# nightgoodl/ovmono3d

Measured on AMD Instinct MI355X. Metric: images/sec/GPU @512x512 DINOv2-L SFP; AP3D delta vs reference, higher is better.
Workload: dtype f16x3; 1 GPU; DINOv2 vitl14 + SFP + ROIHeads3DGDINO (native GroundingDINO Swin-B/BERT-base, 900 queries, 6 categories -> NMS) + ROIAlign + CubeHead + decode, batch 1/GPU, 512x512 synthetic -> network res 532 -> canvas 896 (T=4097), random-init weights (seed 0); precision=f16x3, parallelism=dp1 (image-sharded, no data-path collective)

## Files before the change

### ovmono3d_amd/csrc/attn.hip

```cpp
#include "kernels.hpp"
#include "attn_tail.hpp"
#include <type_traits>

namespace ovm {

__device__ __forceinline__ int swz128(int row, int chunk) { return chunk ^ ((row >> 1) & 7); }

__device__ __forceinline__ void split2_pk(float p0, float p1, uint32_t& hp, uint32_t& lp) {
  float d0, d1;
  asm("s_nop 0\n\tv_cvt_pk_f16_f32 %0, %1, %2" : "=v"(hp) : "v"(p0), "v"(p1));
  asm("v_fma_mix_f32 %0, %1, 1.0, -%2 op_sel:[0,0,0] op_sel_hi:[0,0,1]" : "=v"(d0) : "v"(p0), "v"(hp));
  asm("v_fma_mix_f32 %0, %1, 1.0, -%2 op_sel:[0,0,1] op_sel_hi:[0,0,1]" : "=v"(d1) : "v"(p1), "v"(hp));
  asm("v_cvt_pk_f16_f32 %0, %1, %2" : "=v"(lp) : "v"(d0), "v"(d1));
}
__device__ __forceinline__ uint32_t cvt2_pk(float p0, float p1) {
  uint32_t hp;
  asm("s_nop 0\n\tv_cvt_pk_f16_f32 %0, %1, %2" : "=v"(hp) : "v"(p0), "v"(p1));
  return hp;
}
typedef uint32_t u32x4 __attribute__((ext_vector_type(4)));

template <int N> __device__ __forceinline__ void wait_vmcnt_n() {
  __builtin_amdgcn_s_waitcnt((N & 0xF) | (7 << 4) | (15 << 8) | ((N >> 4) << 14));
}

constexpr float kPShift = 14.0f;

#ifndef OVM_ATTN_ILV
#define OVM_ATTN_ILV 0
#endif
#ifndef OVM_ATTN_RD
#define OVM_ATTN_RD 3
#endif
template <int NPASS, int NW>
__global__ __launch_bounds__(64 * NW, NW == 4 ? 2 : 1) void attn_kernel(const AttnParams p) {
  extern __shared__ __attribute__((aligned(16))) char smem[];
  if ((int)blockIdx.x >= p.main_blocks) { attn_tail_any<NPASS>(p, (int)blockIdx.x - p.main_blocks, smem); return; }
  static_assert(NW == 4 || NW == 8, "4 or 8 waves");
  const unsigned long long t_wg0 = p.stamps ? __builtin_amdgcn_s_memtime() : 0ull;
  constexpr int PART = 64 * 128;
  constexpr int SLOT = PART * ((NPASS == 3) ? 2 : 1);
  constexpr int RD = OVM_ATTN_RD;
  char* const Kring = smem;
  char* const Vring = smem + RD * SLOT;
  const int tid = threadIdx.x, lane = tid & 63, wave = tid >> 6;
  const int nqb = (p.Tq + 32 * NW - 1) / (32 * NW);
  const int bid = xcd_remap(blockIdx.x, p.main_blocks);
  const int bh = bid / nqb, qb = bid - bh * nqb;
  const int b = bh / p.heads, head = bh - b * p.heads;
  const int T = p.T;
  const size_t qk_base = (size_t)bh * T * 64;
  const size_t v_base = (size_t)bh * 64 * p.Tpad;
  const int h = lane >> 5, r = lane & 31;

  int q = qb * (32 * NW) + wave * 32 + r;
  const bool q_ok = q < p.Tq;
  if (!q_ok) q = T - 1;
  half8 qh[4], ql[4];
#pragma unroll
  for (int s = 0; s < 4; ++s) {
    qh[s] = *(const half8*)(p.Qhi + qk_base + (size_t)q * 64 + 16 * s + 8 * h);
    if (NPASS == 3) ql[s] = *(const half8*)(p.Qlo + qk_base + (size_t)q * 64 + 16 * s + 8 * h);
  }

  constexpr int PPW = 8 / NW;
  int drow[PPW], dch[PPW];
#pragma unroll
  for (int t = 0; t < PPW; ++t) {
    drow[t] = (wave + NW * t) * 8 + (lane >> 3);
    dch[t] = swz128(drow[t], lane & 7) * 8;
  }
  auto stageK = [&](int slot, int it) {
    char* base = Kring + slot * SLOT;
    const int k0 = it * 64;
#pragma unroll
    for (int t = 0; t < PPW; ++t) {
      int key = k0 + drow[t]; if (key > T - 1) key = T - 1;
      const size_t o = qk_base + (size_t)key * 64 + dch[t];
      glds16(p.Khi + o, base + (wave + NW * t) * 1024);
      if (NPASS == 3) glds16(p.Klo + o, base + PART + (wave + NW * t) * 1024);
    }
  };
  auto stageV = [&](int slot, int it) {
    char* base = Vring + slot * SLOT;
    const int k0 = it * 64;
#pragma unroll
    for (int t = 0; t < PPW; ++t) {
      const size_t o = v_base + (size_t)drow[t] * p.Tpad + k0 + dch[t];
      glds16(p.Vhi + o, base + (wave + NW * t) * 1024);
      if (NPASS == 3) glds16(p.Vlo + o, base + PART + (wave + NW * t) * 1024);
    }
  };
  auto qk = [&](const char* kb, f32x16* s) {
#if OVM_ATTN_ILV
#pragma unroll
    for (int i = 0; i < 2; ++i)
#pragma unroll
      for (int e = 0; e < 16; ++e) s[i][e] = 0.f;
#pragma unroll
    for (int st = 0; st < 4; ++st) {
      half8 kh[2], kl[2];
#pragma unroll
      for (int i = 0; i < 2; ++i) {
        const int row = 32 * i + r;
        const int off = row * 128 + swz128(row, 2 * st + h) * 16;
        kh[i] = *(const half8*)(kb + off);
        if (NPASS == 3) kl[i] = *(const half8*)(kb + PART + off);
      }
      if (NPASS == 3) {
#pragma unroll
        for (int i = 0; i < 2; ++i) s[i] = __builtin_amdgcn_mfma_f32_32x32x16_f16(kl[i], qh[st], s[i], 0, 0, 0);
#pragma unroll
        for (int i = 0; i < 2; ++i) s[i] = __builtin_amdgcn_mfma_f32_32x32x16_f16(kh[i], ql[st], s[i], 0, 0, 0);
      }
#pragma unroll
      for (int i = 0; i < 2; ++i) s[i] = __builtin_amdgcn_mfma_f32_32x32x16_f16(kh[i], qh[st], s[i], 0, 0, 0);
    }
#else
#pragma unroll
    for (int i = 0; i < 2; ++i) {
#pragma unroll
      for (int e = 0; e < 16; ++e) s[i][e] = 0.f;
      const int row = 32 * i + r;
#pragma unroll
      for (int st = 0; st < 4; ++st) {
        const int off = row * 128 + swz128(row, 2 * st + h) * 16;
        const half8 kh = *(const half8*)(kb + off);
        if (NPASS == 3) {
          const half8 kl = *(const half8*)(kb + PART + off);
          s[i] = __builtin_amdgcn_mfma_f32_32x32x16_f16(kl, qh[st], s[i], 0, 0, 0);
          s[i] = __builtin_amdgcn_mfma_f32_32x32x16_f16(kh, ql[st], s[i], 0, 0, 0);
        }
        s[i] = __builtin_amdgcn_mfma_f32_32x32x16_f16(kh, qh[st], s[i], 0, 0, 0);
      }
    }
#endif
  };

  f32x16 o0[2];
#pragma unroll
  for (int t = 0; t < 2; ++t)
#pragma unroll
    for (int i = 0; i < 16; ++i) o0[t][i] = 0.f;
  float m_run = -1e30f, l_run = 0.f;

  const int nt = (T + 63) >> 6;
  stageK(0, 0);
  stageV(0, 0);
  if (nt > 1) stageK(1, 1);
  if (RD >= 3) {
    if (nt > 2) stageK(2, 2);
    if (nt > 1) stageV(1, 1);
  }
  if (RD >= 4) {
    if (nt > 3) stageK(3, 3);
    if (nt > 2) stageV(2, 2);
  }
  int prev_mine = 0;
  asm volatile("s_waitcnt vmcnt(0)" ::: "memory");
  __syncthreads();
  f32x16 sc[2], sn[2];
  qk(Kring, sc);
  __syncthreads();

  auto tile = [&](int it, auto last_tag) {
    constexpr bool LAST = decltype(last_tag)::value;
    if (!LAST) {
      if (it + RD < nt) stageK(it % RD, it + RD);
      if (it + RD - 1 < nt) stageV((it + RD - 1) % RD, it + RD - 1);
      qk(Kring + ((it + 1) % RD) * SLOT, sn);
    }
    const int kbase = it * 64;
    if (LAST) {
#pragma unroll
      for (int i = 0; i < 2; ++i)
#pragma unroll
        for (int e = 0; e < 16; ++e) {
          const int key = kbase + 32 * i + (e & 3) + 8 * (e >> 2) + 4 * h;
          if (key >= T) sc[i][e] = -1e30f;
        }
    }
    float mx = -1e30f;
#pragma unroll
    for (int i = 0; i < 2; ++i)
#pragma unroll
      for (int e = 0; e < 16; ++e) mx = fmaxf(mx, sc[i][e]);
    mx = fmaxf(mx, __shfl_xor(mx, 32, 64));
    const float m_new = fmaxf(m_run, mx);
    const float alpha = __builtin_amdgcn_exp2f(m_run - m_new);
    m_run = m_new;
    typedef float f32x2 __attribute__((ext_vector_type(2)));
    const f32x2 shift2 = {kPShift - m_new, kPShift - m_new};
    f32x2 psum2 = {0.f, 0.f};
    u32x4 phu[2][2], plu[2][2];
#pragma unroll
    for (int i = 0; i < 2; ++i)
#pragma unroll
      for (int sp = 0; sp < 2; ++sp) {
#pragma unroll
        for (int e = 0; e < 8; e += 2) {
          f32x2 d = {sc[i][8 * sp + e], sc[i][8 * sp + e + 1]};
          d += shift2;
// ... 22 lines not shown
          const int off = row * 128 + swz128(row, 4 * i + 2 * sp + h) * 16;
          vh[t] = *(const half8*)(vb + off);
          if (NPASS == 3) vl[t] = *(const half8*)(vb + PART + off);
        }
        if (NPASS == 3) {
#pragma unroll
          for (int t = 0; t < 2; ++t) o0[t] = __builtin_amdgcn_mfma_f32_32x32x16_f16(vl[t], __builtin_bit_cast(half8, phu[i][sp]), o0[t], 0, 0, 0);
#pragma unroll
          for (int t = 0; t < 2; ++t) o0[t] = __builtin_amdgcn_mfma_f32_32x32x16_f16(vh[t], __builtin_bit_cast(half8, plu[i][sp]), o0[t], 0, 0, 0);
        }
#pragma unroll
        for (int t = 0; t < 2; ++t) o0[t] = __builtin_amdgcn_mfma_f32_32x32x16_f16(vh[t], __builtin_bit_cast(half8, phu[i][sp]), o0[t], 0, 0, 0);
      }
#else
#pragma unroll
    for (int t = 0; t < 2; ++t) {
      const int row = 32 * t + r;
#pragma unroll
      for (int i = 0; i < 2; ++i)
#pragma unroll
        for (int sp = 0; sp < 2; ++sp) {
          const int off = row * 128 + swz128(row, 4 * i + 2 * sp + h) * 16;
          const half8 vh = *(const half8*)(vb + off);
          if (NPASS == 3) {
            const half8 vl = *(const half8*)(vb + PART + off);
            o0[t] = __builtin_amdgcn_mfma_f32_32x32x16_f16(vl, __builtin_bit_cast(half8, phu[i][sp]), o0[t], 0, 0, 0);
            o0[t] = __builtin_amdgcn_mfma_f32_32x32x16_f16(vh, __builtin_bit_cast(half8, plu[i][sp]), o0[t], 0, 0, 0);
          }
          o0[t] = __builtin_amdgcn_mfma_f32_32x32x16_f16(vh, __builtin_bit_cast(half8, phu[i][sp]), o0[t], 0, 0, 0);
        }
    }
#endif
    if (!LAST) {
      if (RD >= 3) {
        constexpr int PP = PPW * ((NPASS == 3) ? 2 : 1);
        const int mine = ((it + RD < nt) ? PP : 0) + ((it + RD - 1 < nt) ? PP : 0);
        const int allow = mine + ((RD >= 4) ? prev_mine : 0);
        prev_mine = mine;
        if (allow >= 4 * PP) __builtin_amdgcn_s_waitcnt((4 * PP) | (7 << 4) | (15 << 8));
        else if (allow == 3 * PP) __builtin_amdgcn_s_waitcnt((3 * PP) | (7 << 4) | (15 << 8));
        else if (allow == 2 * PP) __builtin_amdgcn_s_waitcnt((2 * PP) | (7 << 4) | (15 << 8));
        else if (allow == PP) __builtin_amdgcn_s_waitcnt(PP | (7 << 4) | (15 << 8));
        else __builtin_amdgcn_s_waitcnt(0 | (7 << 4) | (15 << 8));
        asm volatile("s_waitcnt lgkmcnt(0)" ::: "memory");
        __builtin_amdgcn_s_barrier();
      } else {
        asm volatile("s_waitcnt vmcnt(0)" ::: "memory");
        __syncthreads();
      }
      sc[0] = sn[0];
      sc[1] = sn[1];
    }
  };
  for (int it = 0; it + 1 < nt; ++it) tile(it, std::false_type{});
  tile(nt - 1, std::true_type{});

  const float l_tot = l_run + __shfl_xor(l_run, 32, 64);
  const float inv = 1.0f / l_tot;
  if (q_ok) {
    const size_t orow = ((size_t)b * T + q) * p.ldo + (p.o_il ? head * 128 : head * 64);
#pragma unroll
    for (int t = 0; t < 2; ++t)
#pragma unroll
      for (int g = 0; g < 4; ++g) {
        half4 hv, lv;
#pragma unroll
        for (int e = 0; e < 4; ++e) {
// ... 273 lines not shown
  const int b = bh / p.heads, head = bh - b * p.heads;
  const float* recs = p.tail_ws + (size_t)tq * kTailSplit * kTailRec;
  float M = -1e30f;
  for (int i = 0; i < kTailSplit; ++i) M = fmaxf(M, recs[i * kTailRec]);
  float Ltot = 0.f, o = 0.f;
  for (int i = 0; i < kTailSplit; ++i) {
    const float w = __builtin_amdgcn_exp2f(recs[i * kTailRec] - M);
    Ltot = fmaf(recs[i * kTailRec + 1], w, Ltot);
    o = fmaf(recs[i * kTailRec + 4 + tid], w, o);
  }
  half_t hh, ll; split_f16(o / Ltot, hh, ll);
  const size_t oo = ((size_t)b * p.T + q) * p.ldo + (p.o_il ? il_col(head * 64 + tid) : head * 64 + tid);
  p.Ohi[oo] = hh;
  if (p.Olo) p.Olo[oo] = ll;
}

static int g_attn_tail = 1;
void attn_set_tail_rows(int on) { g_attn_tail = on; }
static int g_attn_tail_split = 1;
void attn_set_tail_split(int on) { g_attn_tail_split = on; }
size_t attn_tail_ws_floats(int B, int heads) { return (size_t)B * heads * 8 * kTailSplit * kTailRec; }
static int g_attn_lds_pad = 0;
void attn_set_lds_pad(int v) { g_attn_lds_pad = v; }
static unsigned long long* g_attn_stamps = nullptr;
void attn_set_stamps(unsigned long long* p) { g_attn_stamps = p; }
static int g_attn_prio = 0;
void attn_set_prio(int v) { g_attn_prio = v; }
static int g_attn_pp = 0;
void attn_set_pp(int v) { g_attn_pp = v; }
static int g_attn_q64 = 0;
void attn_set_q64(int v) { g_attn_q64 = v; }
static int g_attn_waves = 0;
void attn_set_waves(int v) { g_attn_waves = (v == 4 || v == 8) ? v : 0; }

int launch_attention(const AttnParams& p, int npass, hipStream_t s) {
  if (p.T <= 0 || p.B <= 0) return OVM_OK;
  if (p.Tpad % 64 != 0 || p.Tpad < ((p.T + 63) / 64) * 64) return OVM_ERR_SHAPE;
  if (npass == 3 && (!p.Qlo || !p.Klo || !p.Vlo)) return OVM_ERR_INVALID;
  AttnParams pm = p;
  pm.stamps = g_attn_stamps;
  pm.prio_mode = g_attn_prio;
  const int nw = g_attn_waves ? g_attn_waves : (p.corun ? 4 : 8);
  const int qpb = 32 * nw;
  const int tail = p.T % qpb;
  int tail_blocks = 0;
  pm.Tq = p.T;
  if (g_attn_tail && tail > 0 && tail <= 8 && p.T > qpb && (p.Tpad + 16) * 4 <= 2 * 2 * 64 * 128) {
    pm.Tq = p.T - tail;
    if (!g_attn_tail_split) { pm.tail_ws = nullptr; pm.tail_cnt = nullptr; }
    tail_blocks = tail * p.heads * p.B * (pm.tail_ws ? kTailSplit : 1);
  } else { pm.tail_ws = nullptr; pm.tail_cnt = nullptr; }
  const int nqb = (pm.Tq + qpb - 1) / qpb;
  pm.main_blocks = nqb * p.heads * p.B;
  const dim3 grid(pm.main_blocks + tail_blocks), block(64 * nw);
  const int pad = g_attn_lds_pad;
  if (npass == 3) {
    const int smem = OVM_ATTN_RD * 4 * 64 * 128 + pad;
    if (nw == 8 && g_attn_q64 && !g_attn_pp) {
      const int r64 = launch_attention64(pm, tail_blocks, s);
      if (r64 == OVM_OK && tail_blocks > 0 && pm.tail_ws) hipLaunchKernelGGL(attn_tail_combine_kernel, dim3(tail * p.heads * p.B), dim3(64), 0, s, pm);
      return r64;
    }
    if (nw == 8 && g_attn_pp) {
      constexpr int smem_pp = 2 * 4 * 2 * 64 * 128;
      static bool setpp = false;
      if (!setpp) { (void)hipFuncSetAttribute((const void*)attn_pp_kernel<3>, hipFuncAttributeMaxDynamicSharedMemorySize, 160 * 1024); setpp = true; }
#ifdef OVM_DIAG
      if (pm.stamps) {
        (void)hipFuncSetAttribute((const void*)attn_pp_kernel<3, 1>, hipFuncAttributeMaxDynamicSharedMemorySize, 160 * 1024);
        (void)hipFuncSetAttribute((const void*)attn_pp_kernel<3, 2>, hipFuncAttributeMaxDynamicSharedMemorySize, 160 * 1024);
        (void)hipFuncSetAttribute((const void*)attn_pp_kernel<3, 3>, hipFuncAttributeMaxDynamicSharedMemorySize, 160 * 1024);
        if (g_attn_pp == 2) hipLaunchKernelGGL((attn_pp_kernel<3, 2>), grid, block, smem_pp + 8192, s, pm);
        else if (g_attn_pp == 3) hipLaunchKernelGGL((attn_pp_kernel<3, 3>), grid, block, smem_pp + 8192, s, pm);
        else hipLaunchKernelGGL((attn_pp_kernel<3, 1>), grid, block, smem_pp + 8192, s, pm);
      } else
#endif
      hipLaunchKernelGGL((attn_pp_kernel<3>), grid, block, smem_pp + pad, s, pm);
    } else if (nw == 8) {
      static bool set8 = false;
      if (!set8) { (void)hipFuncSetAttribute((const void*)attn_kernel<3, 8>, hipFuncAttributeMaxDynamicSharedMemorySize, 160 * 1024); set8 = true; }
      hipLaunchKernelGGL((attn_kernel<3, 8>), grid, block, smem, s, pm);
    } else {
      static bool set4 = false;
      if (!set4 || pad > 0) { (void)hipFuncSetAttribute((const void*)attn_kernel<3, 4>, hipFuncAttributeMaxDynamicSharedMemorySize, 160 * 1024); set4 = true; }
      hipLaunchKernelGGL((attn_kernel<3, 4>), grid, block, smem, s, pm);
    }
  } else if (nw == 8) hipLaunchKernelGGL((attn_kernel<1, 8>), grid, block, OVM_ATTN_RD * 2 * 64 * 128, s, pm);
  else hipLaunchKernelGGL((attn_kernel<1, 4>), grid, block, OVM_ATTN_RD * 2 * 64 * 128, s, pm);
  if (tail_blocks > 0 && pm.tail_ws) hipLaunchKernelGGL(attn_tail_combine_kernel, dim3(tail * p.heads * p.B), dim3(64), 0, s, pm);
  return hipGetLastError() == hipSuccess ? OVM_OK : OVM_ERR_HIP;
}

}
```

### ovmono3d_amd/csrc/gemm.hip

```cpp
#include "gemm.hpp"

namespace ovm {

static int g_force_bm = 0;
static int g_tail_rows = 1;
static int g_force_stages = 0;
static int g_splitk = 1;
void gemm_set_splitk(int v) { g_splitk = v; }

void gemm_set_stages(int n) { g_force_stages = n; }
void gemm_set_force_bm(int bm) { g_force_bm = bm; }
void gemm_set_tail_rows(int on) { g_tail_rows = on; }

template <int NPASS, int BK, int BM, int NSTAGE, int EPI, int AMODE, bool AIL = false>
static int launch_one(const GemmParams& p, hipStream_t s) {
  constexpr int smem = NSTAGE * (BM + 128) * BK * 2 * ((NPASS == 3) ? 2 : 1);
  if (p.K % BK != 0) return OVM_ERR_SHAPE;
  GemmParams q = p;
  q.M_total = p.M; q.tail_begin = p.M; q.main_tiles = 0;
  q.ldw = (NPASS == 3) ? 2 * p.K : p.K;
  int tail_blocks = 0;
  const int tail = p.M % 128;
  if (g_tail_rows && tail > 0 && tail <= 8 && p.M > 128 && p.K % 64 == 0) {
    q.tail_begin = p.M - tail;
// ... 51 lines not shown
    }
  }
  int tail_blocks = 0;
  const int tail = p.M % 128;
  if (q.ksplit == 1 && g_tail_rows && tail > 0 && tail <= 8 && p.M > 128 && p.K % 64 == 0) {
    q.tail_begin = p.M - tail;
    q.M = q.tail_begin;
    const int cols = gemm_tail_cols(p.N, EPI);
    q.tail_waves = gemm_tail_waves(cols, 8);
    tail_blocks = tail * ((cols + 4 * q.tail_waves - 1) / (4 * q.tail_waves));
  }
  const int tiles_m = (q.M + 127) / 128;
  const int tiles_n = (p.N + 127) / 128;
  q.main_tiles = tiles_m * tiles_n * q.ksplit;
  static bool attr_set = false;
  if (!attr_set) {
    if (hipFuncSetAttribute((const void*)gemm_ws_kernel<NPASS, BK, NS, EPI, AMODE, AIL>, hipFuncAttributeMaxDynamicSharedMemorySize, smem) != hipSuccess)
      return OVM_ERR_HIP;
    attr_set = true;
  }
  hipLaunchKernelGGL((gemm_ws_kernel<NPASS, BK, NS, EPI, AMODE, AIL>), dim3(q.main_tiles + tail_blocks), dim3(512), smem, s, q);
  if (q.ksplit > 1) {
    const long n = (long)p.M * (p.N / 4);
    hipLaunchKernelGGL((splitk_epilogue_kernel<EPI>), dim3((unsigned)((n + 255) / 256)), dim3(256), 0, s, q);
  }
  return hipGetLastError() == hipSuccess ? OVM_OK : OVM_ERR_HIP;
}

static int pick_bm(const GemmParams& p) {
  (void)p;
  return g_force_bm == 256 ? 256 : 128;
}

template <int EPI, int AMODE>
static int launch_prec(const GemmParams& p, int npass, hipStream_t s) {
  if (p.M <= 0 || p.N <= 0) return OVM_OK;
  const int bm = pick_bm(p);
  const int tail_rows = p.M % 128;
  const long tiles_m = (g_tail_rows && tail_rows > 0 && tail_rows <= 8 && p.M > 128 && p.K % 64 == 0) ? p.M / 128 : (p.M + 127) / 128;
  const long tiles = tiles_m * ((p.N + 127) / 128);
  const int st = g_force_stages ? g_force_stages : (tiles <= 512 ? 6 : 2);
  if (npass == 3 && p.a_il) {
    if (st == 6 || st == 5) return launch_ws<3, 32, 3, EPI, AMODE, true>(p, s);
    return launch_one<3, 32, 128, 2, EPI, AMODE, true>(p, s);
  }
  if (st == 5) return npass == 3 ? launch_ws<3, 32, 4, EPI, AMODE>(p, s) : launch_ws<1, 64, 4, EPI, AMODE>(p, s);
  if (st == 6) return npass == 3 ? launch_ws<3, 32, 3, EPI, AMODE>(p, s) : launch_ws<1, 64, 3, EPI, AMODE>(p, s);
  if (npass == 3) {
    if (bm == 256) return st == 3 ? launch_one<3, 32, 256, 3, EPI, AMODE>(p, s) : launch_one<3, 32, 256, 2, EPI, AMODE>(p, s);
    return st == 3 ? launch_one<3, 32, 128, 3, EPI, AMODE>(p, s) : launch_one<3, 32, 128, 2, EPI, AMODE>(p, s);
  }
  if (bm == 256) return st == 3 ? launch_one<1, 64, 256, 3, EPI, AMODE>(p, s) : launch_one<1, 64, 256, 2, EPI, AMODE>(p, s);
  return st == 3 ? launch_one<1, 64, 128, 3, EPI, AMODE>(p, s) : launch_one<1, 64, 128, 2, EPI, AMODE>(p, s);
}

bool gemm_offsets_fit(const GemmParams& p, int npass, int amode) {
  const uint64_t lim = 1ull << 32;
  const uint64_t ldw = (npass == 3) ? 2ull * p.K : (uint64_t)p.K;
  const uint64_t npad = ((uint64_t)p.N + 255) / 256 * 256;
  if (npad * ldw > lim) return false;
  if (amode == A_CONV3X3) {
    if (p.cH <= 0 || p.cW <= 0 || p.cC <= 0) return false;
    const uint64_t Bn = ((uint64_t)p.M + (uint64_t)p.cH * p.cW - 1) / ((uint64_t)p.cH * p.cW);
    return Bn * (p.cH + 2) * (p.cW + 2) * (uint64_t)p.cC <= (1ull << 31);
  }
  const uint64_t rowlen = (npass == 3 && p.a_il) ? 2ull * p.K : (uint64_t)p.K;
  return (uint64_t)(p.M > 0 ? p.M - 1 : 0) * (uint64_t)p.lda + rowlen <= lim;
}

int launch_gemm(const GemmParams& p, int npass, int epi, int amode, hipStream_t s) {
  if (npass == 3 && (p.Alo == nullptr || p.Wlo == nullptr)) return OVM_ERR_INVALID;
  if (!gemm_offsets_fit(p, npass, amode)) return OVM_ERR_CAPACITY;
  if (amode == A_CONV3X3) {
    if (epi != EPI_STORE) return OVM_ERR_INVALID;
    return launch_prec<EPI_STORE, A_CONV3X3>(p, npass, s);
  }
// ... 16 lines not shown
```

### ovmono3d_amd/csrc/gemm.hpp

```cpp
#pragma once
#include "common.hpp"

namespace ovm {

enum AMode { A_ROWMAJOR = 0, A_CONV3X3 = 1 };
enum Epi { EPI_STORE = 0, EPI_RESID = 1, EPI_GELU = 2, EPI_QKV = 3, EPI_PATCH = 4, EPI_CONVT = 5, EPI_SWIGLU = 6 };

struct GemmParams {
  const half_t* Ahi; const half_t* Alo; int lda;
  const half_t* Whi; const half_t* Wlo;
  int ldw;
  int a_il;
  int ksplit, kchunk; float* part;
  unsigned long long* stamps;
  float* part_ws; size_t part_cap;
  int ws_slot;
  int M, N, K;
  int cH, cW, cC;
  const float* bias;
  const float* gamma;
  float* X; int ldx;
  const int* row_map;
  float* C; int ldc;
  half_t* Ohi; half_t* Olo; int ldo;
// ... 358 lines not shown
#pragma unroll
  for (int mi = 0; mi < 4; ++mi) {
    const int m = m0 + wm * 64 + mi * 16 + fr;
    if (m >= p.M) continue;
    if (EPI == EPI_SWIGLU) {
#pragma unroll
      for (int ni = 0; ni < 4; ni += 2) epilogue_swiglu4(p, m, ((n0 + wn * 64) >> 1) + ni * 8 + fq * 4, acc[ni][mi], acc[ni + 1][mi]);
      continue;
    }
#pragma unroll
    for (int ni = 0; ni < 4; ++ni) {
      const int n = n0 + wn * 64 + ni * 16 + fq * 4;
      epilogue4<EPI>(p, m, n, acc[ni][mi]);
    }
  }
}

template <int N> __device__ __forceinline__ void wait_vmcnt() {
  __builtin_amdgcn_s_waitcnt((N & 0xF) | (7 << 4) | (15 << 8) | ((N >> 4) << 14));
}

template <int NPASS, int BK, int NS, int EPI, int AMODE, bool AIL = false>
__global__ __launch_bounds__(512) void gemm_ws_kernel(const GemmParams p) {
  if ((int)blockIdx.x >= p.main_tiles) { gemm_tail_body<NPASS, EPI, AMODE, AIL>(p, (int)blockIdx.x - p.main_tiles); return; }
  extern __shared__ __attribute__((aligned(16))) char smem[];
  constexpr int BM = 128, NPW = 4;
  using SA = Side<NPASS, BK, AIL && NPASS == 3>;
  using SW = Side<NPASS, BK, NPASS == 3>;
  constexpr int OFF_A = 0, OFF_W = SA::bytes(BM);
  constexpr int STAGE = SA::bytes(BM) + SW::bytes(128);
  constexpr int IA = BM / SA::RPI / NPW;
  constexpr int IW = 128 / SW::RPI / NPW;
  constexpr int PER_STAGE = IA * SA::PARTS + IW * SW::PARTS;
  static_assert(NS >= 3 && NS <= 4 && (NS - 2) * PER_STAGE < 64, "ring depth vs vmcnt range");

  const int tid = threadIdx.x, lane = tid & 63, wave = tid >> 6;
  const int tiles_m = (p.M + BM - 1) / BM;
  const int ksplit = p.ksplit > 1 ? p.ksplit : 1;
  const int tiles = p.main_tiles / ksplit;
  const int tiles_n = tiles / tiles_m;
  const int ks = (int)blockIdx.x / tiles;
  int pid = xcd_remap((int)blockIdx.x - ks * tiles, tiles);
  constexpr int GROUP_M = 8;
  const int in_group = GROUP_M * tiles_n;
  const int gid = pid / in_group;
  const int first_m = gid * GROUP_M;
  const int gsz = (tiles_m - first_m) < GROUP_M ? (tiles_m - first_m) : GROUP_M;
  const int tm = first_m + (pid % in_group) % gsz;
  const int tn = (pid % in_group) / gsz;
  const int m0 = tm * BM, n0 = tn * 128;
  const int nk_all = p.K / BK;
  const int kt0 = (ksplit > 1) ? ks * p.kchunk : 0;
  const int nk = (ksplit > 1) ? ((nk_all - kt0 < p.kchunk) ? nk_all - kt0 : p.kchunk) : nk_all;

  if (wave >= 4) {
    const int pw = wave - 4;
    uint32_t aoff[IA], woff[IW];
#pragma unroll
    for (int t = 0; t < IA; ++t) {
      const int row = (pw + NPW * t) * SA::RPI + lane / SA::CH;
      const int chunk = SA::swz(row, lane % SA::CH);
      int m = m0 + row; if (m > p.M - 1) m = p.M - 1;
      aoff[t] = a_row_off<AMODE, AIL && NPASS == 3>(p, m) + chunk * 8;
    }
#pragma unroll
    for (int t = 0; t < IW; ++t) {
      const int row = (pw + NPW * t) * SW::RPI + lane / SW::CH;
      const int chunk = SW::swz(row, lane % SW::CH);
      woff[t] = (uint32_t)(n0 + row) * (uint32_t)p.ldw + chunk * 8;
    }
    auto stage = [&](int slot, int kt) {
      char* base = smem + slot * STAGE;
      const uint32_t ak = a_k_off<AMODE, AIL && NPASS == 3>(p, (kt0 + kt) * BK);
      const uint32_t wk = (uint32_t)((kt0 + kt) * SW::KSTEP);
#pragma unroll
      for (int t = 0; t < IA; ++t) {
        char* dst = base + OFF_A + (pw + NPW * t) * 1024;
        glds16(p.Ahi + aoff[t] + ak, dst);
        if (SA::PARTS == 2) glds16(p.Alo + aoff[t] + ak, dst + BM * SA::ROWB);
      }
#pragma unroll
      for (int t = 0; t < IW; ++t) {
        char* dst = base + OFF_W + (pw + NPW * t) * 1024;
        glds16(p.Whi + woff[t] + wk, dst);
        if (SW::PARTS == 2) glds16(p.Wlo + woff[t] + wk, dst + 128 * SW::ROWB);
      }
    };
#pragma unroll
    for (int t = 0; t < NS - 1; ++t)
      if (t < nk) stage(t, t);
    int slot_next = NS - 1;
    for (int kt = 0; kt < nk; ++kt) {
      const int ahead = (nk - 1 - kt < NS - 2) ? nk - 1 - kt : NS - 2;
      if (ahead >= 2) wait_vmcnt<2 * PER_STAGE>();
      else if (ahead == 1) wait_vmcnt<PER_STAGE>();
      else wait_vmcnt<0>();
      __builtin_amdgcn_s_barrier();
      if (kt + NS - 1 < nk) stage(slot_next, kt + NS - 1);
      slot_next = (slot_next + 1 == NS) ? 0 : slot_next + 1;
    }
    __builtin_amdgcn_s_barrier();
    return;
  }

  const int wm = wave >> 1, wn = wave & 1;
  const int fr = lane & 15, fq = lane >> 4;
  f32x4 acc[4][4];
#pragma unroll
  for (int i = 0; i < 4; ++i)
#pragma unroll
    for (int j = 0; j < 4; ++j) acc[i][j] = (f32x4){0.f, 0.f, 0.f, 0.f};
  constexpr int NF = 4 * (BK / 32);
  half8 ahA[NF], whA[NF], alA[NF], wlA[NF], ahB[NF], whB[NF], alB[NF], wlB[NF];
  int oah[NF], oal[NF], owh[NF], owl[NF];
#pragma unroll
  for (int kk = 0; kk < BK / 32; ++kk)
#pragma unroll
    for (int i = 0; i < 4; ++i) {
      const int ra = wm * 64 + i * 16 + fr, rw = wn * 64 + i * 16 + fr;
      oah[kk * 4 + i] = OFF_A + SA::frag_hi(ra, kk, fq);
      oal[kk * 4 + i] = OFF_A + SA::frag_lo(BM, ra, kk, fq);
      owh[kk * 4 + i] = OFF_W + SW::frag_hi(rw, kk, fq);
      owl[kk * 4 + i] = OFF_W + SW::frag_lo(128, rw, kk, fq);
    }
#define OVM_WS_READ(S, base)                                                            \
  _Pragma("unroll") for (int f = 0; f < NF; ++f) {                                      \
    ah##S[f] = *(const half8*)((base) + oah[f]);                                        \
// ... 143 lines not shown
#pragma unroll
      for (int j = 0; j < 8; ++j) w[j] = (float)wh[j];
      if (NPASS == 3) {
        const half8 wl = *(const half8*)(p.Wlo + wo);
#pragma unroll
        for (int j = 0; j < 8; ++j) w[j] += (float)wl[j];
      }
#pragma unroll
      for (int j = 0; j < 8; ++j) acc[r] = fmaf(a[j], w[j], acc[r]);
    }
  }
  f32x4 v, u = {0.f, 0.f, 0.f, 0.f};
#pragma unroll
  for (int r = 0; r < 4; ++r) v[r] = wave_sum(acc[r]);
  if (EPI == EPI_SWIGLU) {
#pragma unroll
    for (int r = 0; r < 4; ++r) u[r] = wave_sum(acc[NR - 4 + r]);
  }
  if (lane == 0) {
    GemmParams q = p; q.M = p.M_total;
    if (EPI == EPI_SWIGLU) epilogue_swiglu4(q, m, n, v, u); else epilogue4<EPI>(q, m, n, v);
  }
}

inline int gemm_tail_waves(int N, int max_waves) { int w = max_waves; while (w > 1 && (N + 4 * w - 1) / (4 * w) < 128) w >>= 1; return w; }
int launch_gemm(const GemmParams& p, int npass, int epi, int amode, hipStream_t stream);
bool gemm_offsets_fit(const GemmParams& p, int npass, int amode);
bool gemm256_supported(const GemmParams& p, int npass);
int launch_gemm256(const GemmParams& p, int epi, int ksplit_hint, hipStream_t stream);
void gemm_set_force_bm(int bm);
void gemm_set_tail_rows(int on);
void gemm_set_stages(int n);
void gemm_set_splitk(int v);
bool gemm_small_supported(const float* A, int lda, int K);
int launch_gemm_small(const float* A, int lda, int M, int K, const half_t* Whi, const half_t* Wlo, int N, int Kpad, const float* bias, int act,
                      const float* R, int ldr, float* C, int ldc, int npass, hipStream_t s);
int launch_gemm_small_ex(const float* A, const float* A2, int lda, int M, int K, const half_t* Whi, const half_t* Wlo, int N, int Kpad,
                         const float* bias, int act, const float* R, int ldr, float* C, int ldc, int npass, float* ws, size_t ws_bytes,
                         hipStream_t s);
void gemm_small_set(int target_blocks, int max_ksplit);
void gemm_small_set_stages(int n);
void gemm_small_set_wpe(int n);
void glinear_set_small_max_tiles(int t);
void gbmm_set_tiled(int v);

}
```

### ovmono3d_amd/csrc/kernels.hpp

```cpp
#pragma once
#include "common.hpp"
#include "gemm.hpp"

namespace ovm {

struct ImageDesc {
  const uint8_t* data;
  int H, W;
  int64_t sC, sH, sW;
};

struct LnOut {
  half_t* hi; half_t* lo; int ld;
  float* f32; int ldf;
  int padH, padW;
  int il;
};

struct AttnParams {
  const half_t *Qhi, *Qlo, *Khi, *Klo, *Vhi, *Vlo;
  half_t *Ohi, *Olo; int ldo;
  int o_il;
  int B, heads, T, Tpad;
  int corun;
// ... 28 lines not shown
  const float* scores;
  const int* classes;
  const int* batch_idx;
  const ImageMeta* meta;
  int n; float virtual_focal;
  int postprocess;
  float* rec;
  int* keep;
};

int launch_patch_gather(const ImageDesc* d_imgs, int B, int G, int patch, int Kpad, const float* mean, const float* stdv,
                        half_t* Ahi, half_t* Alo, hipStream_t s);
struct TowerViews;
int launch_patch_gather_f32(const TowerViews& v, int B, int G, int Kpad, half_t* Ahi, half_t* Alo, hipStream_t s);
int launch_ln_gelu_split(half_t* hi, half_t* lo, int M, int D, const float* gamma, const float* beta, float eps, hipStream_t s);
int launch_cls_init(float* X, const float* cls, const float* pos, const float* reg, int R, int B, int T, int D, hipStream_t s);
int launch_ln_rows(const float* X, int ldx, int M, int D, const float* gamma, const float* beta, float eps,
                   const LnOut& o, hipStream_t s);
int launch_tokens_cast(const float* X, int B, int T, int G2, int D, int ldo, const float* depth_tok,
                       half_t* Ohi, half_t* Olo, hipStream_t s);
int launch_tokens_writeback(float* X, const float* F, int B, int T, int G2, int D, hipStream_t s);
int launch_maxpool2(const half_t* Ihi, const half_t* Ilo, int B, int G, int D, half_t* Ohi, half_t* Olo, hipStream_t s);
int launch_depth_resize(const float* Dp, int B, int Hd, int Wd, int G, float* out, hipStream_t s);
int launch_resize_bilinear_f32(const float* src, int B, int Hd, int Wd, int Ho, int Wo, float* out, hipStream_t s);
int launch_zero(void* p, size_t bytes, hipStream_t s);
int launch_attention(const AttnParams& p, int npass, hipStream_t s);
int launch_attention64(const AttnParams& pm, int tail_blocks, hipStream_t s);
void attn_set_q64(int v);
void attn_set_tail_split(int on);
size_t attn_tail_ws_floats(int B, int heads);
void attn_set_tail_rows(int on);
void attn_set_lds_pad(int v);
void attn_set_waves(int v);
void attn_set_pp(int v);
void attn_set_prio(int v);
void attn_set_stamps(unsigned long long* p);
int launch_roi_align(const RoiParams& p, hipStream_t s);
int launch_cube_decode(const CubeDecodeParams& p, hipStream_t s);
int launch_compact_records(const float* rec, const int* keep, int n, int B, float* out, int* counts, hipStream_t s);

}
```

### ovmono3d_amd/csrc/ops.hip

```cpp
#include <hip/hip_runtime.h>
#include <cstring>
#include <vector>
#include "../../include/ovm3d.h"
#include "kernels.hpp"
#include "det2d.hpp"
#include "gdino.hpp"
#include "tower.hpp"

using namespace ovm;

namespace {
__global__ void split_kernel(const float* __restrict__ x, int64_t n, half_t* __restrict__ hi, half_t* __restrict__ lo) {
  const int64_t i = (int64_t)blockIdx.x * blockDim.x + threadIdx.x;
  if (i >= n) return;
  half_t h, l; split_f16(x[i], h, l);
  hi[i] = h;
  if (lo) lo[i] = l;
}
__global__ void qkv_layout_kernel(const float* __restrict__ qkv, int B, int T, int Tpad, int heads,
                                  half_t* Qh, half_t* Ql, half_t* Kh, half_t* Kl, half_t* Vh, half_t* Vl) {
  const int D = heads * 64;
  const int64_t i = (int64_t)blockIdx.x * blockDim.x + threadIdx.x;
  const int64_t total = (int64_t)B * T * 3 * D;
  if (i >= total) return;
// ... 336 lines not shown
  if (!views || B < 1 || B > kMaxTowerViews) return OVM_ERR_INVALID;
  TowerViews v; memset(&v, 0, sizeof(v));
  v.n = B;
  for (int b = 0; b < B; ++b) v.v[b] = TowerView{(const float*)(uintptr_t)views[4 * b], views[4 * b + 1], views[4 * b + 2], views[4 * b + 3]};
  return launch_patch_gather_f32(v, B, G, Kpad, (half_t*)hi, (half_t*)lo, (hipStream_t)stream);
}

int ovm_op_cls_init(float* X, const float* cls, const float* pos, const float* reg, int32_t R, int32_t B, int32_t T, int32_t D,
                    ovm_stream_t stream) {
  return launch_cls_init(X, cls, pos, reg, R, B, T, D, (hipStream_t)stream);
}

int ovm_op_tokens_cast(const float* X, int32_t B, int32_t T, int32_t G2, int32_t D, int32_t ldo, const float* depth_tok, uint16_t* hi,
                       uint16_t* lo, ovm_stream_t stream) {
  return launch_tokens_cast(X, B, T, G2, D, ldo, depth_tok, (half_t*)hi, (half_t*)lo, (hipStream_t)stream);
}

int ovm_op_tokens_writeback(float* X, const float* F, int32_t B, int32_t T, int32_t G2, int32_t D, ovm_stream_t stream) {
  return launch_tokens_writeback(X, F, B, T, G2, D, (hipStream_t)stream);
}

int ovm_op_maxpool2(const uint16_t* in_hi, const uint16_t* in_lo, int32_t B, int32_t G, int32_t D, uint16_t* out_hi, uint16_t* out_lo,
                    ovm_stream_t stream) {
  return launch_maxpool2((const half_t*)in_hi, (const half_t*)in_lo, B, G, D, (half_t*)out_hi, (half_t*)out_lo, (hipStream_t)stream);
}

int ovm_tune_set(const char* key, int32_t value) {
  if (!key) return OVM_ERR_INVALID;
  ovm::bump_tune_generation();
  if (!strcmp(key, "gemm_bm")) { gemm_set_force_bm(value); return OVM_OK; }
  if (!strcmp(key, "gemm_stages")) { gemm_set_stages(value); return OVM_OK; }
  if (!strcmp(key, "gemm_splitk")) { gemm_set_splitk(value); return OVM_OK; }
  if (!strcmp(key, "gemm_tail")) { gemm_set_tail_rows(value); return OVM_OK; }
  if (!strcmp(key, "attn_waves")) { attn_set_waves(value); return OVM_OK; }
  if (!strcmp(key, "attn_pp")) {
#ifndef OVM_DIAG
    if (value < 0 || value > 1) return OVM_ERR_INVALID;
#endif
    attn_set_pp(value); return OVM_OK;
  }
  if (!strcmp(key, "gdino_mlp_fused")) { ovm::set_gdino_mlp_fused(value); return OVM_OK; }
  if (!strcmp(key, "gdino_enc_fold")) { ovm::set_gdino_enc_fold(value); return OVM_OK; }
  if (!strcmp(key, "gdino_enc_tap")) { ovm::set_gdino_enc_tap(value); return OVM_OK; }
  if (!strcmp(key, "gdino_text_cache")) { ovm::set_gdino_text_cache(value); return OVM_OK; }
  if (!strcmp(key, "gdino_ffn_split")) { ovm::set_gdino_ffn_split(value); return OVM_OK; }
  if (!strcmp(key, "gdino_swin_tap")) { ovm::set_gdino_swin_tap(value); return OVM_OK; }
  if (!strcmp(key, "gdino_swin_fused")) { ovm::set_gdino_swin_fused(value); return OVM_OK; }
  if (!strcmp(key, "gdino_gemm256")) { ovm::set_gdino_gemm256(value); return OVM_OK; }
  if (!strcmp(key, "gdino_dec_chain")) { ovm::set_gdino_dec_chain(value); return OVM_OK; }
  if (!strcmp(key, "msdeform_vec")) { msdeform_set_vec(value); return OVM_OK; }
  if (!strcmp(key, "attn_q64")) { attn_set_q64(value); return OVM_OK; }
  if (!strcmp(key, "attn_prio")) { attn_set_prio(value); return OVM_OK; }
  if (!strcmp(key, "attn_lds_pad")) { attn_set_lds_pad(value); return OVM_OK; }
  if (!strcmp(key, "attn_tail")) { attn_set_tail_rows(value); return OVM_OK; }
  if (!strcmp(key, "attn_tail_split")) { attn_set_tail_split(value); return OVM_OK; }
  if (!strcmp(key, "glin_small_max_tiles")) { glinear_set_small_max_tiles(value); return OVM_OK; }
  if (!strcmp(key, "glin_target_blocks")) { gemm_small_set(value, -1); return OVM_OK; }
  if (!strcmp(key, "gbmm_tiled")) { gbmm_set_tiled(value); return OVM_OK; }
  if (!strcmp(key, "glin_stages")) { gemm_small_set_stages(value); return OVM_OK; }
  if (!strcmp(key, "glin_wpe")) { gemm_small_set_wpe(value); return OVM_OK; }
  if (!strcmp(key, "glin_max_ksplit")) { gemm_small_set(-1, value); return OVM_OK; }
  if (!strcmp(key, "gemm256_ksplit")) { ovm::set_gemm256_ksplit(value); return OVM_OK; }
  if (!strcmp(key, "gemm256_n192")) { ovm::gemm256_set_n192(value); return OVM_OK; }
  if (!strcmp(key, "gemm256")) { ovm::set_use_gemm256(value); return OVM_OK; }
  if (!strcmp(key, "op_gemm256")) { g_op_gemm256 = value; return OVM_OK; }
  if (!strcmp(key, "gdino_branches")) { ovm::set_gdino_branches(value); return OVM_OK; }
// ... 85 lines not shown
```

Before: 56.14 images/sec.

## Stage attention K/V tiles through registers and allow deeper GEMM ring

Adds a register-staged variant of the flash attention kernel, enabled by default. Each wave loads the next K/V tiles from global memory into registers and writes them to the LDS ring one iteration later, replacing direct global-to-LDS loads and their vmcnt bookkeeping. The goal is to overlap global latency with the MFMA work, at the cost of more VGPRs, which may reduce occupancy or cause spills. It also adds an optional 4- or 5-slot ring for the warp-specialized GEMM, off by default.

```diff
diff --git a/ovmono3d_amd/csrc/attn.hip b/ovmono3d_amd/csrc/attn.hip
--- a/ovmono3d_amd/csrc/attn.hip
+++ b/ovmono3d_amd/csrc/attn.hip
@@ -32,7 +32,7 @@
 #ifndef OVM_ATTN_RD
 #define OVM_ATTN_RD 3
 #endif
-template <int NPASS, int NW>
+template <int NPASS, int NW, bool STG = false>
 __global__ __launch_bounds__(64 * NW, NW == 4 ? 2 : 1) void attn_kernel(const AttnParams p) {
   extern __shared__ __attribute__((aligned(16))) char smem[];
   if ((int)blockIdx.x >= p.main_blocks) { attn_tail_any<NPASS>(p, (int)blockIdx.x - p.main_blocks, smem); return; }
@@ -91,6 +91,33 @@
       if (NPASS == 3) glds16(p.Vlo + o, base + PART + (wave + NW * t) * 1024);
     }
   };
+  auto ld_k = [&](int it, half8* kh, half8* kl) {
+    const int k0 = it * 64;
+#pragma unroll
+    for (int t = 0; t < PPW; ++t) {
+      int key = k0 + drow[t]; if (key > T - 1) key = T - 1;
+      const size_t o = qk_base + (size_t)key * 64 + dch[t];
+      kh[t] = *(const half8*)(p.Khi + o);
+      if (NPASS == 3) kl[t] = *(const half8*)(p.Klo + o);
+    }
+  };
+  auto ld_v = [&](int it, half8* vh, half8* vl) {
+    const int k0 = it * 64;
+#pragma unroll
+    for (int t = 0; t < PPW; ++t) {
+      const size_t o = v_base + (size_t)drow[t] * p.Tpad + k0 + dch[t];
+      vh[t] = *(const half8*)(p.Vhi + o);
+      if (NPASS == 3) vl[t] = *(const half8*)(p.Vlo + o);
+    }
+  };
+  auto wr_tile = [&](char* base, const half8* hi, const half8* lo) {
+#pragma unroll
+    for (int t = 0; t < PPW; ++t) {
+      char* dst = base + (wave + NW * t) * 1024 + lane * 16;
+      *(half8*)dst = hi[t];
+      if (NPASS == 3) *(half8*)(dst + PART) = lo[t];
+    }
+  };
   auto qk = [&](const char* kb, f32x16* s) {
 #if OVM_ATTN_ILV
 #pragma unroll
@@ -145,29 +172,56 @@
   float m_run = -1e30f, l_run = 0.f;
 
   const int nt = (T + 63) >> 6;
-  stageK(0, 0);
-  stageV(0, 0);
-  if (nt > 1) stageK(1, 1);
-  if (RD >= 3) {
-    if (nt > 2) stageK(2, 2);
-    if (nt > 1) stageV(1, 1);
-  }
-  if (RD >= 4) {
-    if (nt > 3) stageK(3, 3);
-    if (nt > 2) stageV(2, 2);
-  }
+  half8 pkh[PPW], pkl[PPW], pvh[PPW], pvl[PPW];
   int prev_mine = 0;
-  asm volatile("s_waitcnt vmcnt(0)" ::: "memory");
-  __syncthreads();
+  if (STG) {
+    static_assert(!STG || RD == 3, "register staging is written for the 3-slot rings");
+    {
+      half8 ah[PPW], al[PPW], bh[PPW], bl[PPW], ch[PPW], cl[PPW], dh[PPW], dl[PPW], eh[PPW], el[PPW];
+      const int t1 = nt > 1 ? 1 : nt - 1, t2 = nt > 2 ? 2 : nt - 1;
+      ld_k(0, ah, al); ld_v(0, bh, bl); ld_k(t1, ch, cl); ld_k(t2, dh, dl); ld_v(t1, eh, el);
+      ld_k(nt > RD ? RD : nt - 1, pkh, pkl);
+      ld_v(nt > RD - 1 ? RD - 1 : nt - 1, pvh, pvl);
+      wr_tile(Kring, ah, al); wr_tile(Vring, bh, bl); wr_tile(Kring + SLOT, ch, cl); wr_tile(Kring + 2 * SLOT, dh, dl);
+      wr_tile(Vring + SLOT, eh, el);
+    }
+    asm volatile("s_waitcnt lgkmcnt(0)" ::: "memory");
+    __builtin_amdgcn_s_barrier();
+  } else {
+    stageK(0, 0);
+    stageV(0, 0);
+    if (nt > 1) stageK(1, 1);
+    if (RD >= 3) {
+      if (nt > 2) stageK(2, 2);
+      if (nt > 1) stageV(1, 1);
+    }
+    if (RD >= 4) {
+      if (nt > 3) stageK(3, 3);
+      if (nt > 2) stageV(2, 2);
+    }
+    asm volatile("s_waitcnt vmcnt(0)" ::: "memory");
+    __syncthreads();
+  }
   f32x16 sc[2], sn[2];
   qk(Kring, sc);
-  __syncthreads();
+  if (STG) { asm volatile("s_waitcnt lgkmcnt(0)" ::: "memory"); __builtin_amdgcn_s_barrier(); }
+  else __syncthreads();
 
   auto tile = [&](int it, auto last_tag) {
     constexpr bool LAST = decltype(last_tag)::value;
     if (!LAST) {
-      if (it + RD < nt) stageK(it % RD, it + RD);
-      if (it + RD - 1 < nt) stageV((it + RD - 1) % RD, it + RD - 1);
+      if (STG) {
+        if (it + RD < nt) wr_tile(Kring + (it % RD) * SLOT, pkh, pkl);
+        if (it + RD - 1 < nt) wr_tile(Vring + ((it + RD - 1) % RD) * SLOT, pvh, pvl);
+      } else {
+        if (it + RD < nt) stageK(it % RD, it + RD);
+        if (it + RD - 1 < nt) stageV((it + RD - 1) % RD, it + RD - 1);
+      }
+      if (STG) {
+        ld_k(it + RD + 1 < nt ? it + RD + 1 : nt - 1, pkh, pkl);
+        ld_v(it + RD < nt ? it + RD : nt - 1, pvh, pvl);
+        __builtin_amdgcn_sched_barrier(0);
+      }
       qk(Kring + ((it + 1) % RD) * SLOT, sn);
     }
     const int kbase = it * 64;
@@ -256,7 +310,10 @@
     }
 #endif
     if (!LAST) {
-      if (RD >= 3) {
+      if (STG) {
+        asm volatile("s_waitcnt lgkmcnt(0)" ::: "memory");
+        __builtin_amdgcn_s_barrier();
+      } else if (RD >= 3) {
         constexpr int PP = PPW * ((NPASS == 3) ? 2 : 1);
         const int mine = ((it + RD < nt) ? PP : 0) + ((it + RD - 1 < nt) ? PP : 0);
         const int allow = mine + ((RD >= 4) ? prev_mine : 0);
@@ -596,6 +653,19 @@
 void attn_set_q64(int v) { g_attn_q64 = v; }
 static int g_attn_waves = 0;
 void attn_set_waves(int v) { g_attn_waves = (v == 4 || v == 8) ? v : 0; }
+static int g_attn_stage = 1;
+int attn_set_stage(int v) {
+  if (v < 0 || v > 1) return OVM_ERR_INVALID;
+  g_attn_stage = v;
+  return OVM_OK;
+}
+
+template <int NPASS, int NW, bool STG>
+static void launch_attn_kernel(const AttnParams& pm, dim3 grid, int smem, hipStream_t s) {
+  static bool set = false;
+  if (!set) { (void)hipFuncSetAttribute((const void*)attn_kernel<NPASS, NW, STG>, hipFuncAttributeMaxDynamicSharedMemorySize, 160 * 1024); set = true; }
+  hipLaunchKernelGGL((attn_kernel<NPASS, NW, STG>), grid, dim3(64 * NW), smem, s, pm);
+}
 
 int launch_attention(const AttnParams& p, int npass, hipStream_t s) {
   if (p.T <= 0 || p.B <= 0) return OVM_OK;
@@ -641,16 +711,15 @@
 #endif
       hipLaunchKernelGGL((attn_pp_kernel<3>), grid, block, smem_pp + pad, s, pm);
     } else if (nw == 8) {
-      static bool set8 = false;
-      if (!set8) { (void)hipFuncSetAttribute((const void*)attn_kernel<3, 8>, hipFuncAttributeMaxDynamicSharedMemorySize, 160 * 1024); set8 = true; }
-      hipLaunchKernelGGL((attn_kernel<3, 8>), grid, block, smem, s, pm);
+      if (g_attn_stage) launch_attn_kernel<3, 8, true>(pm, grid, smem, s); else launch_attn_kernel<3, 8, false>(pm, grid, smem, s);
     } else {
-      static bool set4 = false;
-      if (!set4 || pad > 0) { (void)hipFuncSetAttribute((const void*)attn_kernel<3, 4>, hipFuncAttributeMaxDynamicSharedMemorySize, 160 * 1024); set4 = true; }
-      hipLaunchKernelGGL((attn_kernel<3, 4>), grid, block, smem, s, pm);
-    }
-  } else if (nw == 8) hipLaunchKernelGGL((attn_kernel<1, 8>), grid, block, OVM_ATTN_RD * 2 * 64 * 128, s, pm);
-  else hipLaunchKernelGGL((attn_kernel<1, 4>), grid, block, OVM_ATTN_RD * 2 * 64 * 128, s, pm);
+      if (g_attn_stage) launch_attn_kernel<3, 4, true>(pm, grid, smem, s); else launch_attn_kernel<3, 4, false>(pm, grid, smem, s);
+    }
+  } else {
+    const int smem1 = OVM_ATTN_RD * 2 * 64 * 128;
+    if (nw == 8) { if (g_attn_stage) launch_attn_kernel<1, 8, true>(pm, grid, smem1, s); else launch_attn_kernel<1, 8, false>(pm, grid, smem1, s); }
+    else { if (g_attn_stage) launch_attn_kernel<1, 4, true>(pm, grid, smem1, s); else launch_attn_kernel<1, 4, false>(pm, grid, smem1, s); }
+  }
   if (tail_blocks > 0 && pm.tail_ws) hipLaunchKernelGGL(attn_tail_combine_kernel, dim3(tail * p.heads * p.B), dim3(64), 0, s, pm);
   return hipGetLastError() == hipSuccess ? OVM_OK : OVM_ERR_HIP;
 }
diff --git a/ovmono3d_amd/csrc/gemm.hip b/ovmono3d_amd/csrc/gemm.hip
--- a/ovmono3d_amd/csrc/gemm.hip
+++ b/ovmono3d_amd/csrc/gemm.hip
@@ -107,6 +107,14 @@
   return g_force_bm == 256 ? 256 : 128;
 }
 
+static int g_ws_slots = 0;
+int gemm_set_ws_slots(int v) {
+  if (v != 0 && (v < 3 || v > 5)) return OVM_ERR_INVALID;
+  g_ws_slots = v;
+  return OVM_OK;
+}
+static int ws_slots() { return g_ws_slots ? g_ws_slots : 3; }
+
 template <int EPI, int AMODE>
 static int launch_prec(const GemmParams& p, int npass, hipStream_t s) {
   if (p.M <= 0 || p.N <= 0) return OVM_OK;
@@ -116,7 +124,14 @@
   const long tiles = tiles_m * ((p.N + 127) / 128);
   const int st = g_force_stages ? g_force_stages : (tiles <= 512 ? 6 : 2);
   if (npass == 3 && p.a_il) {
-    if (st == 6 || st == 5) return launch_ws<3, 32, 3, EPI, AMODE, true>(p, s);
+    if (st == 6 || st == 5) {
+      if constexpr (AMODE == A_ROWMAJOR) {
+        const int ns = ws_slots();
+        if (ns == 4) return launch_ws<3, 32, 4, EPI, AMODE, true>(p, s);
+        if (ns == 5) return launch_ws<3, 32, 5, EPI, AMODE, true>(p, s);
+      }
+      return launch_ws<3, 32, 3, EPI, AMODE, true>(p, s);
+    }
     return launch_one<3, 32, 128, 2, EPI, AMODE, true>(p, s);
   }
   if (st == 5) return npass == 3 ? launch_ws<3, 32, 4, EPI, AMODE>(p, s) : launch_ws<1, 64, 4, EPI, AMODE>(p, s);
diff --git a/ovmono3d_amd/csrc/gemm.hpp b/ovmono3d_amd/csrc/gemm.hpp
--- a/ovmono3d_amd/csrc/gemm.hpp
+++ b/ovmono3d_amd/csrc/gemm.hpp
@@ -414,7 +414,8 @@
   constexpr int IA = BM / SA::RPI / NPW;
   constexpr int IW = 128 / SW::RPI / NPW;
   constexpr int PER_STAGE = IA * SA::PARTS + IW * SW::PARTS;
-  static_assert(NS >= 3 && NS <= 4 && (NS - 2) * PER_STAGE < 64, "ring depth vs vmcnt range");
+  static_assert(NS >= 3 && NS <= 5 && (NS - 2) * PER_STAGE < 64, "ring depth vs vmcnt range");
+  static_assert(NS * STAGE <= 160 * 1024 && 4 * 64 * 68 * 4 <= NS * STAGE, "ring and epilogue tiles vs the LDS");
 
   const int tid = threadIdx.x, lane = tid & 63, wave = tid >> 6;
   const int tiles_m = (p.M + BM - 1) / BM;
@@ -474,7 +475,8 @@
     int slot_next = NS - 1;
     for (int kt = 0; kt < nk; ++kt) {
       const int ahead = (nk - 1 - kt < NS - 2) ? nk - 1 - kt : NS - 2;
-      if (ahead >= 2) wait_vmcnt<2 * PER_STAGE>();
+      if (NS >= 5 && ahead >= 3) wait_vmcnt<3 * PER_STAGE>();
+      else if (ahead >= 2) wait_vmcnt<2 * PER_STAGE>();
       else if (ahead == 1) wait_vmcnt<PER_STAGE>();
       else wait_vmcnt<0>();
       __builtin_amdgcn_s_barrier();
@@ -684,6 +686,7 @@
 void gemm_set_tail_rows(int on);
 void gemm_set_stages(int n);
 void gemm_set_splitk(int v);
+int gemm_set_ws_slots(int v);
 bool gemm_small_supported(const float* A, int lda, int K);
 int launch_gemm_small(const float* A, int lda, int M, int K, const half_t* Whi, const half_t* Wlo, int N, int Kpad, const float* bias, int act,
                       const float* R, int ldr, float* C, int ldc, int npass, hipStream_t s);
diff --git a/ovmono3d_amd/csrc/kernels.hpp b/ovmono3d_amd/csrc/kernels.hpp
--- a/ovmono3d_amd/csrc/kernels.hpp
+++ b/ovmono3d_amd/csrc/kernels.hpp
@@ -84,6 +84,7 @@
 void attn_set_tail_rows(int on);
 void attn_set_lds_pad(int v);
 void attn_set_waves(int v);
+int attn_set_stage(int v);
 void attn_set_pp(int v);
 void attn_set_prio(int v);
 void attn_set_stamps(unsigned long long* p);
diff --git a/ovmono3d_amd/csrc/ops.hip b/ovmono3d_amd/csrc/ops.hip
--- a/ovmono3d_amd/csrc/ops.hip
+++ b/ovmono3d_amd/csrc/ops.hip
@@ -392,6 +392,8 @@
   if (!strcmp(key, "gemm_stages")) { gemm_set_stages(value); return OVM_OK; }
   if (!strcmp(key, "gemm_splitk")) { gemm_set_splitk(value); return OVM_OK; }
   if (!strcmp(key, "gemm_tail")) { gemm_set_tail_rows(value); return OVM_OK; }
+  if (!strcmp(key, "gemm_ws_slots")) return gemm_set_ws_slots(value);
+  if (!strcmp(key, "attn_stage")) return attn_set_stage(value);
   if (!strcmp(key, "attn_waves")) { attn_set_waves(value); return OVM_OK; }
   if (!strcmp(key, "attn_pp")) {
 #ifndef OVM_DIAG
```

Result: no change. 56.55 images/sec (median of 6 runs) (+0.7%).
